# smpurkis/PyTorch-Face-Detection-from-Scratch

Hardware: AMD Instinct MI355X
Metric: train imgs/sec (PoolResnet 480^2, bs=256 per GPU) (higher is better)
Workload: dtype f32 (3x3 convs: bf16x3 split MFMA, fp32 accumulate)

## Files before the change

pytorch-face-detection-from-scratch_amd/csrc/fdet_wgrad3x3_ps.hip:

```cpp
#include "fdet_conv3x3_x3.h"
#include "fdet_ps.h"
#include "fdet_ldsdma.h"
#include <algorithm>

using namespace fdet;

typedef __attribute__((address_space(3))) void* lds_void_t;
typedef const __attribute__((address_space(1))) void* glb_void_t;
typedef short s16x4 __attribute__((ext_vector_type(4)));
typedef __attribute__((address_space(3))) s16x4* lds_s16x4_t;
typedef __bf16 bf16x2_t __attribute__((ext_vector_type(2)));
typedef unsigned u32x2_t __attribute__((ext_vector_type(2)));
typedef unsigned u32x4_t __attribute__((ext_vector_type(4)));

namespace {

#ifndef WG_DBG
#define WG_DBG 0
#endif
constexpr int WG_MAXL = 16;
constexpr int XL = 5, ZL = 3;
constexpr int XA = XL * 64 + 4;
constexpr int ZLS = 66;
constexpr int ZA = 212;
constexpr int WG_LDS_UNITS = 16 * XA + 16 * ZA;

struct PsWgArgs {
  const bf16x8* x[WG_MAXL];
  const bf16x8* dz[WG_MAXL];
  float* ws;
  float* wsb;
  int plane, img;
  int lpi, real_lpi, nlines;
  int nslab, lpw;
  unsigned magic_lpi;
};

__device__ __forceinline__ bf16x2_t as_bf16x2(unsigned u) { return __builtin_bit_cast(bf16x2_t, u); }
__device__ __forceinline__ u32x2_t tr2(const char* base, int off) {
  return __builtin_bit_cast(u32x2_t, __builtin_amdgcn_ds_read_tr16_b64_v4i16((lds_s16x4_t)(base + off)));
}
__host__ __device__ constexpr int x_line(int S, int ky, int WP) { return 16 * S + (ky - 1) * WP < 0 ? 0 : (16 * S + (ky - 1) * WP >= 64 ? 2 : 1); }
__host__ __device__ constexpr int x_off(int S, int ky, int WP) {
  return 16 * S + (ky - 1) * WP < 0 ? 16 * S + (ky - 1) * WP + 64 : (16 * S + (ky - 1) * WP >= 64 ? 16 * S + (ky - 1) * WP - 64 : 16 * S + (ky - 1) * WP);
}

template <int WP, bool FL1, bool P16 = false>
__global__ void __launch_bounds__(256, 1)
k_wgrad3x3_ps(const PsWgArgs a) {
  extern __shared__ __attribute__((aligned(16))) char smem[];
  bf16x8* const lds = reinterpret_cast<bf16x8*>(smem);
  const int tid = threadIdx.x, lane = tid & 63;
  const int wid = __builtin_amdgcn_readfirstlane(tid >> 6);
  const int m = wid & 1, j = wid >> 1;
  const int layer = blockIdx.y;
  const bf16x8* __restrict__ gx = a.x[layer];
  const bf16x8* __restrict__ gz = a.dz[layer];
  {
    f32x4* z = reinterpret_cast<f32x4*>(smem);
    for (int t = tid; t < WG_LDS_UNITS; t += 256) z[t] = f32x4{0.f, 0.f, 0.f, 0.f};
  }
  const int i16 = lane & 15, g16 = (lane >> 4) & 1, kh = lane >> 5;
  const int q = i16 >> 2, pp = i16 & 3;
  const int GA = 4 * m + 2 * g16 + (pp >> 1), GB = 4 * j + 2 * g16 + (pp >> 1);
  const int lane_x = (GB * XA + 8 * kh + q) * 16 + (pp & 1) * 8;
  const int lane_z = (16 * XA + GA * ZA + 1 + 8 * kh + q) * 16 + (pp & 1) * 8;
  constexpr int XPL = 8 * XA * 16, ZPL = 8 * ZA * 16;

  const int l0 = blockIdx.x * a.lpw, l1 = min(l0 + a.lpw, a.nlines);
  f32x16 acc[9];
#pragma unroll
  for (int t = 0; t < 9; ++t)
#pragma unroll
    for (int r = 0; r < 16; ++r) acc[t][r] = 0.f;
  float bsum = 0.f;
  const unsigned bsel0 = j == 0 ? 0x3f803f80u : 0u, bsel1 = j == 1 ? 0x3f803f80u : 0u;

  const unsigned lds0 = (unsigned)(size_t)(lds_void_t)smem;
  const unsigned tbytes = (unsigned)((a.nlines / a.lpi) + 2) * (unsigned)a.img * 16u;
  const dma_u32x4 xrs = dma_rsrc(gx - a.img, tbytes), zrs = dma_rsrc(gz - a.img, tbytes);
  const unsigned lane16 = (unsigned)lane * 16u;
#define WG_PIECE(RS, LG, AI, DST)                                                                  \
  {                                                                                                \
    const int lg_ = (LG) + a.lpi;                                                                  \
    const int n_ = (int)__umulhi((unsigned)lg_, a.magic_lpi);                                      \
    const unsigned so_ = (unsigned)(n_ * a.img + ((AI) >> 3) * a.plane + ((AI) & 7) * (a.lpi * 64) + (lg_ - n_ * a.lpi) * 64) * 16u; \
    dma_piece(lds0 + (unsigned)(DST) * 16u, lane16, RS, so_);                                      \
  }
#define WG_ISSUE(LX, SX, LZ, SZ)                                                                   \
  if (!(P16 && wid >= 2)) {                                   \
    _Pragma("unroll") for (int k_ = 0; k_ < 4; ++k_) {                                             \
      const int ai_ = 4 * wid + k_;                                                                \
      WG_PIECE(xrs, LX, ai_, ai_ * XA + (SX) * 64)                                                  \
      WG_PIECE(zrs, LZ, ai_, 16 * XA + ai_ * ZA + (SZ) * ZLS + 1)                                   \
    }                                                                                              \
  }
  __syncthreads();
  int sx = ((l0 - 1) % XL + XL) % XL, sz = l0 % ZL;
#define XS(D) ((sx + (D)) % XL)
  WG_ISSUE(l0 - 1, XS(0), l0, sz)
  WG_ISSUE(l0, XS(1), l0 + 1, (sz + 1) % ZL)
  if (!(P16 && wid >= 2)) {
    _Pragma("unroll") for (int k_ = 0; k_ < 4; ++k_) {
      const int ai_ = 4 * wid + k_;
      WG_PIECE(xrs, l0 + 1, ai_, ai_ * XA + XS(2) * 64)
      WG_PIECE(xrs, l0 + 2, ai_, ai_ * XA + XS(3) * 64)
    }
  }
  asm volatile("s_waitcnt vmcnt(0)" ::: "memory");

  u32x4_t zf[2][3][2], xf[2][3][2];
#define WG_FRAGS(F, S, ZB, XB0, XB1, XB2)                                                          \
  {                                                                                                \
    _Pragma("unroll") for (int k_ = 0; k_ < 3; ++k_)                                               \
      _Pragma("unroll") for (int pl_ = 0; pl_ < (P16 ? 1 : 2); ++pl_)                              \
        _Pragma("unroll") for (int h_ = 0; h_ < 2; ++h_) {                                         \
          const u32x2_t z_ = (WG_DBG & 4) ? u32x2_t{0x3f803f80u + (unsigned)lane, 0x40004000u} : tr2(ZB, pl_ * ZPL + (16 * (S) + 4 * h_ - (k_ - 1)) * 16); \
          zf[F][k_][pl_][2 * h_] = z_[0]; zf[F][k_][pl_][2 * h_ + 1] = z_[1];                      \
          const char* xb_ = x_line((S), k_, WP) == 0 ? XB0 : (x_line((S), k_, WP) == 1 ? XB1 : XB2); \
          const u32x2_t x_ = (WG_DBG & 4) ? u32x2_t{0x3f803f80u, 0x40004000u + (unsigned)lane} : tr2(xb_, pl_ * XPL + (x_off((S), k_, WP) + 4 * h_) * 16); \
          xf[F][k_][pl_][2 * h_] = x_[0]; xf[F][k_][pl_][2 * h_ + 1] = x_[1];                      \
        }                                                                                          \
  }
  int band = l0;
  if (FL1) {
    __builtin_amdgcn_s_barrier();
    const char* zb_ = smem + lane_z + sz * (ZLS * 16);
    const char* xb0 = smem + lane_x + XS(0) * 1024;
    const char* xb1 = smem + lane_x + XS(1) * 1024;
    const char* xb2 = smem + lane_x + XS(2) * 1024;
    WG_FRAGS(0, 0, zb_, xb0, xb1, xb2)
  }
  int row = l0 - (l0 / a.lpi) * a.lpi;
  while (band < l1) {
  const int n_full = row < a.real_lpi ? min(l1 - band, a.real_lpi - row) : 0;
  row += n_full;
  for (const int bend = band + n_full; band < bend; ++band) {
    if (FL1) asm volatile("s_waitcnt vmcnt(0)" ::: "memory");
    else asm volatile("s_waitcnt vmcnt(8)" ::: "memory");
    __builtin_amdgcn_s_barrier();
    if (!(WG_DBG & 1)) WG_ISSUE(band + 3, XS(4), band + 2, (sz + 2) % ZL)
    __builtin_amdgcn_sched_barrier(0);
    {
      const char* zb_ = smem + lane_z + sz * (ZLS * 16);
      const char* xb0 = smem + lane_x + XS(0) * 1024;
      const char* xb1 = smem + lane_x + XS(1) * 1024;
      const char* xb2 = smem + lane_x + XS(2) * 1024;
      const char* zbn = smem + lane_z + ((sz + 1) % ZL) * (ZLS * 16);
      const char* xb3 = smem + lane_x + XS(3) * 1024;
      if (!FL1) {
        WG_FRAGS(0, 0, zb_, xb0, xb1, xb2)
        __builtin_amdgcn_sched_barrier(0);
      }
#pragma unroll
      for (int s = 0; s < 4; ++s) {
        const int F = s & 1;
        if (s < 3) WG_FRAGS(F ^ 1, s + 1, zb_, xb0, xb1, xb2)
        else if (FL1) WG_FRAGS(0, 0, zbn, xb1, xb2, xb3)
#pragma unroll
        for (int ky = 0; ky < 3; ++ky)
#pragma unroll
          for (int kx = 0; kx < 3; ++kx) {
            const int t = ky * 3 + kx;
            const bf16x8 ah = __builtin_bit_cast(bf16x8, zf[F][kx][0]), al = __builtin_bit_cast(bf16x8, zf[F][kx][1]);
            const bf16x8 bh = __builtin_bit_cast(bf16x8, xf[F][ky][0]), bl = __builtin_bit_cast(bf16x8, xf[F][ky][1]);
            if (!(WG_DBG & 2)) {
              if (!P16) {
                acc[t] = __builtin_amdgcn_mfma_f32_32x32x16_bf16(ah, bl, acc[t], 0, 0, 0);
                acc[t] = __builtin_amdgcn_mfma_f32_32x32x16_bf16(al, bh, acc[t], 0, 0, 0);
              }
              acc[t] = __builtin_amdgcn_mfma_f32_32x32x16_bf16(ah, bh, acc[t], 0, 0, 0);
            }
          }
        {
          const bf16x2_t sel = as_bf16x2((s & 1) ? bsel1 : bsel0);
#pragma unroll
          for (int pl = 0; pl < (P16 ? 1 : 2); ++pl) {
            const u32x4_t zv = zf[F][1][pl];
            bsum = __builtin_amdgcn_fdot2_f32_bf16(as_bf16x2(zv[0]), sel, bsum, false);
            bsum = __builtin_amdgcn_fdot2_f32_bf16(as_bf16x2(zv[1]), sel, bsum, false);
            bsum = __builtin_amdgcn_fdot2_f32_bf16(as_bf16x2(zv[2]), sel, bsum, false);
            bsum = __builtin_amdgcn_fdot2_f32_bf16(as_bf16x2(zv[3]), sel, bsum, false);
          }
        }
        if ((s < 3 || FL1) && !P16) {
#pragma unroll
          for (int i = 0; i < 24; ++i) {
            __builtin_amdgcn_sched_group_barrier(0x008, 1, 0);
            __builtin_amdgcn_sched_group_barrier(0x100, 1, 0);
          }
          __builtin_amdgcn_sched_group_barrier(0x008, 3, 0);
        } else if (s < 3 || FL1) {
#pragma unroll
          for (int i = 0; i < 9; ++i) {
            __builtin_amdgcn_sched_group_barrier(0x008, 1, 0);
            if (i < 6) __builtin_amdgcn_sched_group_barrier(0x100, 2, 0);
          }
        }
      }
    }
    sx = (sx + 1) % XL;
    sz = (sz + 1) % ZL;
  }
  if (band < l1 && row >= a.real_lpi) {
    const int n_zero = min(l1 - band, a.lpi - row);
    for (const int bend = band + n_zero; band < bend; ++band) {
      asm volatile("s_waitcnt vmcnt(0)" ::: "memory");
      __builtin_amdgcn_s_barrier();
      if (!(WG_DBG & 1)) WG_ISSUE(band + 3, XS(4), band + 2, (sz + 2) % ZL)
      sx = (sx + 1) % XL;
      sz = (sz + 1) % ZL;
    }
    row += n_zero;
    if (row >= a.lpi) row = 0;
    if (FL1 && band < l1) {
      const char* zb_ = smem + lane_z + sz * (ZLS * 16);
      const char* xb0 = smem + lane_x + XS(0) * 1024;
      const char* xb1 = smem + lane_x + XS(1) * 1024;
      const char* xb2 = smem + lane_x + XS(2) * 1024;
      WG_FRAGS(0, 0, zb_, xb0, xb1, xb2)
    }
  }
  }
  asm volatile("s_waitcnt vmcnt(0)" ::: "memory");
#undef WG_FRAGS
#undef XS
#undef WG_ISSUE
#undef WG_PIECE
  const int l31 = lane & 31, half = lane >> 5;
  const size_t s = (size_t)layer * a.nslab + blockIdx.x;
  float* __restrict__ wsl = a.ws + s * 9 * 64 * 64;
#pragma unroll
  for (int t = 0; t < 9; ++t)
#pragma unroll
    for (int r = 0; r < 16; ++r) {
      const int co = 32 * m + (r & 3) + 8 * (r >> 2) + 4 * half;
      wsl[(t * 64 + co) * 64 + 32 * j + l31] = acc[t][r];
    }
  bsum += __shfl_xor(bsum, 32, 64);
  if (half == 0) a.wsb[(s * 2 + j) * 64 + 32 * m + l31] = bsum;
}

struct PsWgRed { float* dW[WG_MAXL]; float* db[WG_MAXL]; };
__global__ void __launch_bounds__(256)
k_wgrad_ps_reduce(const float* __restrict__ ws, const float* __restrict__ wsb, int nslab, const PsWgRed out) {
  __shared__ float part[256];
  const int layer = blockIdx.y;
  const int el = threadIdx.x & 63, q = threadIdx.x >> 6;
  const bool bias_blk = blockIdx.x == 9 * 64;
  const size_t stride = bias_blk ? 128 : 9 * 4096;
  const float* __restrict__ src = bias_blk ? wsb + (size_t)layer * nslab * 128 + el
                                           : ws + (size_t)layer * nslab * 9 * 4096 + (size_t)blockIdx.x * 64 + el;
  float s = 0.f;
  int k = q;
  for (; k + 28 < nslab; k += 32) {
    float v[8];
#pragma unroll
    for (int u = 0; u < 8; ++u) v[u] = src[(size_t)(k + 4 * u) * stride] + (bias_blk ? src[(size_t)(k + 4 * u) * stride + 64] : 0.f);
#pragma unroll
    for (int u = 0; u < 8; ++u) s += v[u];
  }
  for (; k < nslab; k += 4) s += src[(size_t)k * stride] + (bias_blk ? src[(size_t)k * stride + 64] : 0.f);
  part[threadIdx.x] = s;
  __syncthreads();
  if (q == 0) {
    const float r = ((part[el] + part[64 + el]) + part[128 + el]) + part[192 + el];
    if (bias_blk) {
      out.db[layer][el] = r;
    } else {
      const int e = blockIdx.x * 64 + el;
      const int t = e >> 12, co = (e >> 6) & 63, ci = e & 63;
      out.dW[layer][(co * 64 + ci) * 9 + t] = r;
    }
  }
}

int wg_plan(int L, int N, int H, int W, PsGeo& g, int& nslab, int& lpw) {
  PsStrips sp;
  if (!ps_geo_strips(N, 64, H, W, g, sp) || L < 1 || L > WG_MAXL) return 0;
  const int lpi = g.HP * g.WP / 64;
  const long nlines = (long)g.N * lpi;
  if (nlines + 2 * lpi >= (1 << 20) || (size_t)(g.N + 2) * g.img * 16 >= ((size_t)1 << 32)) return 0;
  nslab = std::max(1, std::min((int)nlines, num_cus() / L));
  lpw = (int)((nlines + nslab - 1) / nslab);
  nslab = (int)((nlines + lpw - 1) / lpw);
  return 1;
}

}

extern "C" size_t fdet_conv3x3_wgrad_ps_ws_bytes(int L, int N, int C, int H, int W) {
  PsGeo g;
  int nslab = 0, lpw = 0;
  if (C != 64 || !wg_plan(L, N, H, W, g, nslab, lpw)) return 0;
  return (size_t)L * nslab * (9 * 4096 + 128) * sizeof(float);
}

namespace {
int wgrad_ps_run(const void* const* h_x, const void* const* h_dz, float* const* h_dW, float* const* h_db, int L, int N, int C,
                 int H, int W, void* ws, size_t ws_bytes, void* stream, bool p16) {
  PsGeo g;
  int nslab = 0, lpw = 0;
  FDET_REQUIRE(h_x && h_dz && h_dW && h_db && ws, "conv3x3_wgrad_ps: null pointer");
  FDET_REQUIRE(C == 64 && wg_plan(L, N, H, W, g, nslab, lpw), "conv3x3_wgrad_ps: unsupported shape (L=%d N=%d C=%d H=%d W=%d)", L, N, C, H, W);
  const size_t need = (size_t)L * nslab * (9 * 4096 + 128) * sizeof(float);
  FDET_REQUIRE(ws_bytes >= need, "conv3x3_wgrad_ps: workspace of %zu bytes needed, %zu given", need, ws_bytes);
  PsWgArgs a;
  PsWgRed red;
  for (int l = 0; l < L; ++l) {
    FDET_REQUIRE(h_x[l] && h_dz[l] && h_dW[l] && h_db[l], "conv3x3_wgrad_ps: null pointer in layer %d", l);
    a.x[l] = reinterpret_cast<const bf16x8*>(h_x[l]);
    a.dz[l] = reinterpret_cast<const bf16x8*>(h_dz[l]);
    red.dW[l] = h_dW[l];
    red.db[l] = h_db[l];
  }
  a.ws = reinterpret_cast<float*>(ws);
  a.wsb = a.ws + (size_t)L * nslab * 9 * 4096;
  a.plane = g.plane; a.img = g.img;
  a.lpi = g.HP * g.WP / 64;
  a.real_lpi = (H * g.WP + 63) / 64;
  a.nlines = g.N * a.lpi;
  a.nslab = nslab; a.lpw = lpw;
  a.magic_lpi = magic_of(a.lpi);
  const size_t lds = (size_t)WG_LDS_UNITS * 16;
  hipStream_t st = (hipStream_t)stream;
  static const bool fl1 = [] { const char* e = getenv("FDET_WGPS_FLIGHT"); return !(e && e[0] == '2'); }();
  auto go = [&](auto kern, bool& done) -> int {
    if (!done) {
      if (hipFuncSetAttribute((const void*)kern, hipFuncAttributeMaxDynamicSharedMemorySize, (int)lds) != hipSuccess) {
        (void)hipGetLastError();
        return fail(FDET_ELAUNCH, "conv3x3_wgrad_ps: cannot reserve %zu bytes of LDS", lds);
      }
      done = true;
    }
    hipLaunchKernelGGL(kern, dim3(nslab, L), dim3(256), lds, st, a);
    return FDET_OK;
  };
  static bool d64a = false, d64b = false, d32a = false, d32b = false, d16a = false, d16b = false, d64p = false, d32p = false, d16p = false;
  int rc0;
  if (p16) {
    if (g.WP == 64) rc0 = go(k_wgrad3x3_ps<64, true, true>, d64p);
    else if (g.WP == 16) rc0 = go(k_wgrad3x3_ps<16, true, true>, d16p);
    else rc0 = go(k_wgrad3x3_ps<32, true, true>, d32p);
  }
  else if (g.WP == 64) rc0 = fl1 ? go(k_wgrad3x3_ps<64, true>, d64a) : go(k_wgrad3x3_ps<64, false>, d64b);
  else if (g.WP == 16) rc0 = fl1 ? go(k_wgrad3x3_ps<16, true>, d16a) : go(k_wgrad3x3_ps<16, false>, d16b);
  else rc0 = fl1 ? go(k_wgrad3x3_ps<32, true>, d32a) : go(k_wgrad3x3_ps<32, false>, d32b);
  if (rc0 != FDET_OK) return rc0;
  int rc = check_launch("fdet_conv3x3_wgrad_ps_batched");
  if (rc != FDET_OK) return rc;
  hipLaunchKernelGGL(k_wgrad_ps_reduce, dim3(9 * 64 + 1, L), dim3(256), 0, st, a.ws, a.wsb, nslab, red);
  return check_launch("fdet_conv3x3_wgrad_ps_batched(reduce)");
}
}

extern "C" int fdet_conv3x3_wgrad_ps_batched(const void* const* h_x, const void* const* h_dz, float* const* h_dW,
                                             float* const* h_db, int L, int N, int C, int H, int W, void* ws,
                                             size_t ws_bytes, void* stream) {
  return wgrad_ps_run(h_x, h_dz, h_dW, h_db, L, N, C, H, W, ws, ws_bytes, stream, false);
}

extern "C" int fdet_conv3x3_wgrad_ps_batched_p16(const void* const* h_x, const void* const* h_dz, float* const* h_dW,
                                                 float* const* h_db, int L, int N, int C, int H, int W, void* ws,
                                                 size_t ws_bytes, void* stream) {
  return wgrad_ps_run(h_x, h_dz, h_dW, h_db, L, N, C, H, W, ws, ws_bytes, stream, true);
}
```

Measured before the change: 92230.

## Split wgrad K-steps across two 4-wave groups with LDS accumulator combine

The block grows from 256 to 512 threads. Two groups of four waves each process alternate 16-column sub-steps of every band (S0/S1) and share the DMA issue work, two pieces per wave instead of four. At the end, group 1 writes its accumulators and bias sums to LDS and group 0 adds them before storing to the workspace. The MFMA/LDS-read interleave is also rewritten as explicit per-tap reads of the next step's fragments with single (not double) fragment buffers. The aim is more latency hiding per CU, at the cost of an extra LDS combine, a larger LDS footprint, and removal of the two-band flight variant.

Result: no change. 92600, median of 6 (+0.4%).

```diff
diff --git a/pytorch-face-detection-from-scratch_amd/csrc/fdet_wgrad3x3_ps.hip b/pytorch-face-detection-from-scratch_amd/csrc/fdet_wgrad3x3_ps.hip
--- a/pytorch-face-detection-from-scratch_amd/csrc/fdet_wgrad3x3_ps.hip
+++ b/pytorch-face-detection-from-scratch_amd/csrc/fdet_wgrad3x3_ps.hip
@@ -24,6 +24,8 @@
 constexpr int ZLS = 66;
 constexpr int ZA = 212;
 constexpr int WG_LDS_UNITS = 16 * XA + 16 * ZA;
+constexpr int WG_CMB_BYTES = 4 * 144 * 64 * 4;
+constexpr int WG_LDS_BYTES = WG_CMB_BYTES + 4 * 64 * 4 > WG_LDS_UNITS * 16 ? WG_CMB_BYTES + 4 * 64 * 4 : WG_LDS_UNITS * 16;
 
 struct PsWgArgs {
   const bf16x8* x[WG_MAXL];
@@ -45,20 +47,16 @@
   return 16 * S + (ky - 1) * WP < 0 ? 16 * S + (ky - 1) * WP + 64 : (16 * S + (ky - 1) * WP >= 64 ? 16 * S + (ky - 1) * WP - 64 : 16 * S + (ky - 1) * WP);
 }
 
-template <int WP, bool FL1, bool P16 = false>
-__global__ void __launch_bounds__(256, 1)
-k_wgrad3x3_ps(const PsWgArgs a) {
-  extern __shared__ __attribute__((aligned(16))) char smem[];
-  bf16x8* const lds = reinterpret_cast<bf16x8*>(smem);
-  const int tid = threadIdx.x, lane = tid & 63;
-  const int wid = __builtin_amdgcn_readfirstlane(tid >> 6);
-  const int m = wid & 1, j = wid >> 1;
+template <int WP, bool P16, int G>
+__device__ __forceinline__ void wg_run(const PsWgArgs& a, char* const smem, const int wid, const int lane) {
+  const int tid = wid * 64 + lane;
+  const int m = wid & 1, j = (wid >> 1) & 1;
   const int layer = blockIdx.y;
   const bf16x8* __restrict__ gx = a.x[layer];
   const bf16x8* __restrict__ gz = a.dz[layer];
   {
     f32x4* z = reinterpret_cast<f32x4*>(smem);
-    for (int t = tid; t < WG_LDS_UNITS; t += 256) z[t] = f32x4{0.f, 0.f, 0.f, 0.f};
+    for (int t = tid; t < WG_LDS_UNITS; t += 512) z[t] = f32x4{0.f, 0.f, 0.f, 0.f};
   }
   const int i16 = lane & 15, g16 = (lane >> 4) & 1, kh = lane >> 5;
   const int q = i16 >> 2, pp = i16 & 3;
@@ -66,6 +64,7 @@
   const int lane_x = (GB * XA + 8 * kh + q) * 16 + (pp & 1) * 8;
   const int lane_z = (16 * XA + GA * ZA + 1 + 8 * kh + q) * 16 + (pp & 1) * 8;
   constexpr int XPL = 8 * XA * 16, ZPL = 8 * ZA * 16;
+  constexpr int S0 = 2 * G, S1 = 2 * G + 1;
 
   const int l0 = blockIdx.x * a.lpw, l1 = min(l0 + a.lpw, a.nlines);
   f32x16 acc[9];
@@ -88,9 +87,9 @@
     dma_piece(lds0 + (unsigned)(DST) * 16u, lane16, RS, so_);                                      \
   }
 #define WG_ISSUE(LX, SX, LZ, SZ)                                                                   \
-  if (!(P16 && wid >= 2)) {                                   \
-    _Pragma("unroll") for (int k_ = 0; k_ < 4; ++k_) {                                             \
-      const int ai_ = 4 * wid + k_;                                                                \
+  if (!(P16 && G == 1)) {                                     \
+    _Pragma("unroll") for (int k_ = 0; k_ < 2; ++k_) {                                             \
+      const int ai_ = 2 * wid + k_;                                                                \
       WG_PIECE(xrs, LX, ai_, ai_ * XA + (SX) * 64)                                                  \
       WG_PIECE(zrs, LZ, ai_, 16 * XA + ai_ * ZA + (SZ) * ZLS + 1)                                   \
     }                                                                                              \
@@ -100,44 +99,74 @@
 #define XS(D) ((sx + (D)) % XL)
   WG_ISSUE(l0 - 1, XS(0), l0, sz)
   WG_ISSUE(l0, XS(1), l0 + 1, (sz + 1) % ZL)
-  if (!(P16 && wid >= 2)) {
-    _Pragma("unroll") for (int k_ = 0; k_ < 4; ++k_) {
-      const int ai_ = 4 * wid + k_;
+  if (!(P16 && G == 1)) {
+    _Pragma("unroll") for (int k_ = 0; k_ < 2; ++k_) {
+      const int ai_ = 2 * wid + k_;
       WG_PIECE(xrs, l0 + 1, ai_, ai_ * XA + XS(2) * 64)
       WG_PIECE(xrs, l0 + 2, ai_, ai_ * XA + XS(3) * 64)
     }
   }
   asm volatile("s_waitcnt vmcnt(0)" ::: "memory");
 
-  u32x4_t zf[2][3][2], xf[2][3][2];
-#define WG_FRAGS(F, S, ZB, XB0, XB1, XB2)                                                          \
+  u32x4_t zf[3][2], xf[3][2];
+#define WG_RZ(K, S, ZB)                                                                            \
+  _Pragma("unroll") for (int pl_ = 0; pl_ < (P16 ? 1 : 2); ++pl_)                                  \
+    _Pragma("unroll") for (int h_ = 0; h_ < 2; ++h_) {                                             \
+      const u32x2_t z_ = (WG_DBG & 4) ? u32x2_t{0x3f803f80u + (unsigned)lane, 0x40004000u} : tr2(ZB, pl_ * ZPL + (16 * (S) + 4 * h_ - ((K) - 1)) * 16); \
+      zf[K][pl_][2 * h_] = z_[0]; zf[K][pl_][2 * h_ + 1] = z_[1];                                  \
+    }
+#define WG_RX(K, S, XB0, XB1, XB2)                                                                 \
+  _Pragma("unroll") for (int pl_ = 0; pl_ < (P16 ? 1 : 2); ++pl_)                                  \
+    _Pragma("unroll") for (int h_ = 0; h_ < 2; ++h_) {                                             \
+      const char* xb_ = x_line((S), (K), WP) == 0 ? XB0 : (x_line((S), (K), WP) == 1 ? XB1 : XB2);  \
+      const u32x2_t x_ = (WG_DBG & 4) ? u32x2_t{0x3f803f80u, 0x40004000u + (unsigned)lane} : tr2(xb_, pl_ * XPL + (x_off((S), (K), WP) + 4 * h_) * 16); \
+      xf[K][pl_][2 * h_] = x_[0]; xf[K][pl_][2 * h_ + 1] = x_[1];                                  \
+    }
+#define WG_FRAGS(S, ZB, XB0, XB1, XB2)                                                             \
+  { WG_RZ(0, S, ZB) WG_RZ(1, S, ZB) WG_RZ(2, S, ZB) WG_RX(0, S, XB0, XB1, XB2) WG_RX(1, S, XB0, XB1, XB2) WG_RX(2, S, XB0, XB1, XB2) }
+#define WG_TAP(KX, KY)                                                                             \
+  if (!(WG_DBG & 2)) {                                                                             \
+    constexpr int t_ = (KY) * 3 + (KX);                                                            \
+    const bf16x8 ah_ = __builtin_bit_cast(bf16x8, zf[KX][0]), bh_ = __builtin_bit_cast(bf16x8, xf[KY][0]); \
+    if (!P16) {                                                                                    \
+      const bf16x8 al_ = __builtin_bit_cast(bf16x8, zf[KX][1]), bl_ = __builtin_bit_cast(bf16x8, xf[KY][1]); \
+      acc[t_] = __builtin_amdgcn_mfma_f32_32x32x16_bf16(ah_, bl_, acc[t_], 0, 0, 0);               \
+      acc[t_] = __builtin_amdgcn_mfma_f32_32x32x16_bf16(al_, bh_, acc[t_], 0, 0, 0);               \
+    }                                                                                              \
+    acc[t_] = __builtin_amdgcn_mfma_f32_32x32x16_bf16(ah_, bh_, acc[t_], 0, 0, 0);                 \
+  }
+#define WG_STEP(S, NS, NZB, NX0, NX1, NX2)                                                            \
   {                                                                                                \
-    _Pragma("unroll") for (int k_ = 0; k_ < 3; ++k_)                                               \
-      _Pragma("unroll") for (int pl_ = 0; pl_ < (P16 ? 1 : 2); ++pl_)                              \
-        _Pragma("unroll") for (int h_ = 0; h_ < 2; ++h_) {                                         \
-          const u32x2_t z_ = (WG_DBG & 4) ? u32x2_t{0x3f803f80u + (unsigned)lane, 0x40004000u} : tr2(ZB, pl_ * ZPL + (16 * (S) + 4 * h_ - (k_ - 1)) * 16); \
-          zf[F][k_][pl_][2 * h_] = z_[0]; zf[F][k_][pl_][2 * h_ + 1] = z_[1];                      \
-          const char* xb_ = x_line((S), k_, WP) == 0 ? XB0 : (x_line((S), k_, WP) == 1 ? XB1 : XB2); \
-          const u32x2_t x_ = (WG_DBG & 4) ? u32x2_t{0x3f803f80u, 0x40004000u + (unsigned)lane} : tr2(xb_, pl_ * XPL + (x_off((S), k_, WP) + 4 * h_) * 16); \
-          xf[F][k_][pl_][2 * h_] = x_[0]; xf[F][k_][pl_][2 * h_ + 1] = x_[1];                      \
-        }                                                                                          \
+    const bf16x2_t sel_ = as_bf16x2(((S) & 1) ? bsel1 : bsel0);                                    \
+    _Pragma("unroll") for (int pl_ = 0; pl_ < (P16 ? 1 : 2); ++pl_) {                              \
+      const u32x4_t zv_ = zf[1][pl_];                                                              \
+      bsum = __builtin_amdgcn_fdot2_f32_bf16(as_bf16x2(zv_[0]), sel_, bsum, false);                \
+      bsum = __builtin_amdgcn_fdot2_f32_bf16(as_bf16x2(zv_[1]), sel_, bsum, false);                \
+      bsum = __builtin_amdgcn_fdot2_f32_bf16(as_bf16x2(zv_[2]), sel_, bsum, false);                \
+      bsum = __builtin_amdgcn_fdot2_f32_bf16(as_bf16x2(zv_[3]), sel_, bsum, false);                \
+    }                                                                                              \
+    WG_TAP(0, 0) WG_TAP(0, 1) WG_TAP(1, 0) WG_TAP(1, 1)                                            \
+    WG_TAP(0, 2) __builtin_amdgcn_sched_barrier(0); WG_RZ(0, NS, NZB)                       \
+    WG_TAP(1, 2) __builtin_amdgcn_sched_barrier(0); WG_RZ(1, NS, NZB)                       \
+    WG_TAP(2, 0) __builtin_amdgcn_sched_barrier(0); WG_RX(0, NS, NX0, NX1, NX2)             \
+    WG_TAP(2, 1) __builtin_amdgcn_sched_barrier(0); WG_RX(1, NS, NX0, NX1, NX2)             \
+    WG_TAP(2, 2) __builtin_amdgcn_sched_barrier(0); WG_RZ(2, NS, NZB) WG_RX(2, NS, NX0, NX1, NX2)  \
   }
   int band = l0;
-  if (FL1) {
+  {
     __builtin_amdgcn_s_barrier();
     const char* zb_ = smem + lane_z + sz * (ZLS * 16);
     const char* xb0 = smem + lane_x + XS(0) * 1024;
     const char* xb1 = smem + lane_x + XS(1) * 1024;
     const char* xb2 = smem + lane_x + XS(2) * 1024;
-    WG_FRAGS(0, 0, zb_, xb0, xb1, xb2)
+    WG_FRAGS(S0, zb_, xb0, xb1, xb2)
   }
   int row = l0 - (l0 / a.lpi) * a.lpi;
   while (band < l1) {
   const int n_full = row < a.real_lpi ? min(l1 - band, a.real_lpi - row) : 0;
   row += n_full;
   for (const int bend = band + n_full; band < bend; ++band) {
-    if (FL1) asm volatile("s_waitcnt vmcnt(0)" ::: "memory");
-    else asm volatile("s_waitcnt vmcnt(8)" ::: "memory");
+    asm volatile("s_waitcnt vmcnt(0)" ::: "memory");
     __builtin_amdgcn_s_barrier();
     if (!(WG_DBG & 1)) WG_ISSUE(band + 3, XS(4), band + 2, (sz + 2) % ZL)
     __builtin_amdgcn_sched_barrier(0);
@@ -148,56 +177,8 @@
       const char* xb2 = smem + lane_x + XS(2) * 1024;
       const char* zbn = smem + lane_z + ((sz + 1) % ZL) * (ZLS * 16);
       const char* xb3 = smem + lane_x + XS(3) * 1024;
-      if (!FL1) {
-        WG_FRAGS(0, 0, zb_, xb0, xb1, xb2)
-        __builtin_amdgcn_sched_barrier(0);
-      }
-#pragma unroll
-      for (int s = 0; s < 4; ++s) {
-        const int F = s & 1;
-        if (s < 3) WG_FRAGS(F ^ 1, s + 1, zb_, xb0, xb1, xb2)
-        else if (FL1) WG_FRAGS(0, 0, zbn, xb1, xb2, xb3)
-#pragma unroll
-        for (int ky = 0; ky < 3; ++ky)
-#pragma unroll
-          for (int kx = 0; kx < 3; ++kx) {
-            const int t = ky * 3 + kx;
-            const bf16x8 ah = __builtin_bit_cast(bf16x8, zf[F][kx][0]), al = __builtin_bit_cast(bf16x8, zf[F][kx][1]);
-            const bf16x8 bh = __builtin_bit_cast(bf16x8, xf[F][ky][0]), bl = __builtin_bit_cast(bf16x8, xf[F][ky][1]);
-            if (!(WG_DBG & 2)) {
-              if (!P16) {
-                acc[t] = __builtin_amdgcn_mfma_f32_32x32x16_bf16(ah, bl, acc[t], 0, 0, 0);
-                acc[t] = __builtin_amdgcn_mfma_f32_32x32x16_bf16(al, bh, acc[t], 0, 0, 0);
-              }
-              acc[t] = __builtin_amdgcn_mfma_f32_32x32x16_bf16(ah, bh, acc[t], 0, 0, 0);
-            }
-          }
-        {
-          const bf16x2_t sel = as_bf16x2((s & 1) ? bsel1 : bsel0);
-#pragma unroll
-          for (int pl = 0; pl < (P16 ? 1 : 2); ++pl) {
-            const u32x4_t zv = zf[F][1][pl];
-            bsum = __builtin_amdgcn_fdot2_f32_bf16(as_bf16x2(zv[0]), sel, bsum, false);
-            bsum = __builtin_amdgcn_fdot2_f32_bf16(as_bf16x2(zv[1]), sel, bsum, false);
-            bsum = __builtin_amdgcn_fdot2_f32_bf16(as_bf16x2(zv[2]), sel, bsum, false);
-            bsum = __builtin_amdgcn_fdot2_f32_bf16(as_bf16x2(zv[3]), sel, bsum, false);
-          }
-        }
-        if ((s < 3 || FL1) && !P16) {
-#pragma unroll
-          for (int i = 0; i < 24; ++i) {
-            __builtin_amdgcn_sched_group_barrier(0x008, 1, 0);
-            __builtin_amdgcn_sched_group_barrier(0x100, 1, 0);
-          }
-          __builtin_amdgcn_sched_group_barrier(0x008, 3, 0);
-        } else if (s < 3 || FL1) {
-#pragma unroll
-          for (int i = 0; i < 9; ++i) {
-            __builtin_amdgcn_sched_group_barrier(0x008, 1, 0);
-            if (i < 6) __builtin_amdgcn_sched_group_barrier(0x100, 2, 0);
-          }
-        }
-      }
+      WG_STEP(S0, S1, zb_, xb0, xb1, xb2)
+      WG_STEP(S1, S0, zbn, xb1, xb2, xb3)
     }
     sx = (sx + 1) % XL;
     sz = (sz + 1) % ZL;
@@ -213,32 +194,67 @@
     }
     row += n_zero;
     if (row >= a.lpi) row = 0;
-    if (FL1 && band < l1) {
+    if (band < l1) {
       const char* zb_ = smem + lane_z + sz * (ZLS * 16);
       const char* xb0 = smem + lane_x + XS(0) * 1024;
       const char* xb1 = smem + lane_x + XS(1) * 1024;
       const char* xb2 = smem + lane_x + XS(2) * 1024;
-      WG_FRAGS(0, 0, zb_, xb0, xb1, xb2)
+      WG_FRAGS(S0, zb_, xb0, xb1, xb2)
     }
   }
   }
   asm volatile("s_waitcnt vmcnt(0)" ::: "memory");
+  __syncthreads();
+#undef WG_STEP
+#undef WG_TAP
 #undef WG_FRAGS
+#undef WG_RX
+#undef WG_RZ
 #undef XS
 #undef WG_ISSUE
 #undef WG_PIECE
+  f32x4* const cmb = reinterpret_cast<f32x4*>(smem) + (size_t)(wid & 3) * (36 * 64) + lane;
+  float* const cmb_b = reinterpret_cast<float*>(smem + WG_CMB_BYTES) + (wid & 3) * 64 + lane;
+  if (G == 1) {
+#pragma unroll
+    for (int t = 0; t < 9; ++t)
+#pragma unroll
+      for (int r4 = 0; r4 < 4; ++r4)
+        cmb[(t * 4 + r4) * 64] = f32x4{acc[t][4 * r4], acc[t][4 * r4 + 1], acc[t][4 * r4 + 2], acc[t][4 * r4 + 3]};
+    *cmb_b = bsum;
+    __syncthreads();
+    return;
+  }
+  __syncthreads();
   const int l31 = lane & 31, half = lane >> 5;
   const size_t s = (size_t)layer * a.nslab + blockIdx.x;
   float* __restrict__ wsl = a.ws + s * 9 * 64 * 64;
 #pragma unroll
   for (int t = 0; t < 9; ++t)
 #pragma unroll
-    for (int r = 0; r < 16; ++r) {
-      const int co = 32 * m + (r & 3) + 8 * (r >> 2) + 4 * half;
-      wsl[(t * 64 + co) * 64 + 32 * j + l31] = acc[t][r];
-    }
+    for (int r4 = 0; r4 < 4; ++r4) {
+      const f32x4 p = cmb[(t * 4 + r4) * 64];
+#pragma unroll
+      for (int e = 0; e < 4; ++e) {
+        const int r = 4 * r4 + e;
+        const int co = 32 * m + (r & 3) + 8 * (r >> 2) + 4 * half;
+        wsl[(t * 64 + co) * 64 + 32 * j + l31] = acc[t][r] + p[e];
+      }
+    }
+  bsum += *cmb_b;
   bsum += __shfl_xor(bsum, 32, 64);
   if (half == 0) a.wsb[(s * 2 + j) * 64 + 32 * m + l31] = bsum;
+}
+
+template <int WP, bool FL1, bool P16 = false>
+__global__ void __launch_bounds__(512, 1)
+k_wgrad3x3_ps(const PsWgArgs a) {
+  static_assert(FL1, "only the one-band flight exists");
+  extern __shared__ __attribute__((aligned(16))) char smem[];
+  const int lane = threadIdx.x & 63;
+  const int wid = __builtin_amdgcn_readfirstlane(threadIdx.x >> 6);
+  if (wid < 4) wg_run<WP, P16, 0>(a, smem, wid, lane);
+  else wg_run<WP, P16, 1>(a, smem, wid, lane);
 }
 
 struct PsWgRed { float* dW[WG_MAXL]; float* db[WG_MAXL]; };
@@ -322,9 +338,8 @@
   a.nlines = g.N * a.lpi;
   a.nslab = nslab; a.lpw = lpw;
   a.magic_lpi = magic_of(a.lpi);
-  const size_t lds = (size_t)WG_LDS_UNITS * 16;
+  const size_t lds = (size_t)WG_LDS_BYTES;
   hipStream_t st = (hipStream_t)stream;
-  static const bool fl1 = [] { const char* e = getenv("FDET_WGPS_FLIGHT"); return !(e && e[0] == '2'); }();
   auto go = [&](auto kern, bool& done) -> int {
     if (!done) {
       if (hipFuncSetAttribute((const void*)kern, hipFuncAttributeMaxDynamicSharedMemorySize, (int)lds) != hipSuccess) {
@@ -333,19 +348,19 @@
       }
       done = true;
     }
-    hipLaunchKernelGGL(kern, dim3(nslab, L), dim3(256), lds, st, a);
+    hipLaunchKernelGGL(kern, dim3(nslab, L), dim3(512), lds, st, a);
     return FDET_OK;
   };
-  static bool d64a = false, d64b = false, d32a = false, d32b = false, d16a = false, d16b = false, d64p = false, d32p = false, d16p = false;
+  static bool d64 = false, d32 = false, d16 = false, d64p = false, d32p = false, d16p = false;
   int rc0;
   if (p16) {
     if (g.WP == 64) rc0 = go(k_wgrad3x3_ps<64, true, true>, d64p);
     else if (g.WP == 16) rc0 = go(k_wgrad3x3_ps<16, true, true>, d16p);
     else rc0 = go(k_wgrad3x3_ps<32, true, true>, d32p);
   }
-  else if (g.WP == 64) rc0 = fl1 ? go(k_wgrad3x3_ps<64, true>, d64a) : go(k_wgrad3x3_ps<64, false>, d64b);
-  else if (g.WP == 16) rc0 = fl1 ? go(k_wgrad3x3_ps<16, true>, d16a) : go(k_wgrad3x3_ps<16, false>, d16b);
-  else rc0 = fl1 ? go(k_wgrad3x3_ps<32, true>, d32a) : go(k_wgrad3x3_ps<32, false>, d32b);
+  else if (g.WP == 64) rc0 = go(k_wgrad3x3_ps<64, true>, d64);
+  else if (g.WP == 16) rc0 = go(k_wgrad3x3_ps<16, true>, d16);
+  else rc0 = go(k_wgrad3x3_ps<32, true>, d32);
   if (rc0 != FDET_OK) return rc0;
   int rc = check_launch("fdet_conv3x3_wgrad_ps_batched");
   if (rc != FDET_OK) return rc;
```
